# colmap/privacy_preserving_sfm

Hardware: AMD Instinct MI355X
Metric: BA iterations/sec + RANSAC hypotheses/sec, 500 cams / 200k line obs (higher is better)
Workload: dtype f64; 1 GPU; configs[2]: 500 cams / 200k line obs full BA (K1+K2+K3, MFMA Schur solve) on 1xMI355X; cams=500, points=25000, obs=200000, camera_model=SIMPLE_RADIAL, reduced_system=3000, successful_steps=2561, lm_chunk=10, submodels=1, exchange=none (independent sub-models), linear_solver=cholesky (one launch: chain workgroup + task list), cholesky_fallbacks=0

## Files before the change

### privacy_preserving_sfm_amd/csrc/chol_block.hpp

```cpp
#pragma once
#include <type_traits>
#include <utility>

#include "ba_impl.hpp"

namespace ppsfm {

constexpr int kNB = 64;
constexpr int kDeferAbove = 280;
constexpr int kNumCUs = 256;
constexpr int kPanelThreads = 1024;
typedef double v4f64 __attribute__((ext_vector_type(4)));

#ifdef PP_CHOL_TRACE
__device__ long long g_chol_trace[32];
__device__ long long g_chol_trace2[32][128];
__device__ int g_chol_step;
#define PP_CHOL_PHASE(i) do { if (threadIdx.x == 0 && blockIdx.x == 0) { const long long t_ = wall_clock64(); g_chol_trace[i] = t_; g_chol_trace2[i][g_chol_step & 127] = t_; } } while (0)
#define PP_CHOL_STAMP(i) do { if (threadIdx.x == 0) g_chol_trace[i] = wall_clock64(); } while (0)
__device__ int g_chol_exp;
#define PP_EXP(bit) (g_chol_exp & (bit))
__device__ long long g_wave_arrive[12][16];
__device__ long long g_bs_trace[5][128];
#define PP_BS_STAMP(slot, blk) do { if (threadIdx.x == 0) g_bs_trace[slot][(blk) & 127] = wall_clock64(); } while (0)
// ... 3 lines not shown
#define PP_CHOL_LAUNCH(slot, k) do { if (threadIdx.x == 0 && (k) < 64) atomicMax((unsigned long long*)&g_chol_launch[slot][k], (unsigned long long)wall_clock64()); } while (0)
__device__ int g_chol_skip;
#define PP_CHOL_SKIPPED(bit) (g_chol_skip & (1 << (bit)))
__device__ long long g_task_trace[24][128];
__device__ int g_dbg_mismatch[16];
__device__ int g_burn_stop;
__device__ unsigned g_burn_hwid[512];
__device__ long long g_spare_wait[3][128];
__device__ unsigned long long g_wait_missing[128];
__device__ long long g_chain_phase[8][128];
__device__ long long g_chain_clk[128];
#define PP_CHAIN_PHASE(slot, k) do { if (threadIdx.x == 0 && (k) < 128) { g_chain_phase[slot][k] = wall_clock64(); if ((slot) == 0) g_chain_clk[k] = clock64(); } } while (0)
#define PP_TASK_MAX(slot, k) do { if (threadIdx.x == 0 && (k) < 128) atomicMax((unsigned long long*)&g_task_trace[slot][k], (unsigned long long)wall_clock64()); } while (0)
#define PP_TASK_MIN(slot, k) do { if (threadIdx.x == 0 && (k) < 128) atomicMin((unsigned long long*)&g_task_trace[slot][k], (unsigned long long)wall_clock64()); } while (0)
#ifdef PP_CHOL_NO_STAMPS
#undef PP_CHOL_PHASE
#undef PP_CHOL_STAMP
#undef PP_WAVE_ARRIVE
#undef PP_CHOL_LAUNCH
#undef PP_CHAIN_PHASE
#undef PP_TASK_MAX
#undef PP_TASK_MIN
#define PP_TASK_MAX(slot, k) do { } while (0)
#define PP_TASK_MIN(slot, k) do { } while (0)
#define PP_CHAIN_PHASE(slot, k) do { } while (0)
#define PP_CHOL_LAUNCH(slot, k) do { } while (0)
#define PP_CHOL_PHASE(i) do { } while (0)
#define PP_CHOL_STAMP(i) do { } while (0)
#define PP_WAVE_ARRIVE(b) do { } while (0)
#endif
#else
#define PP_BS_STAMP(slot, blk) do { } while (0)
#define PP_TASK_MAX(slot, k) do { } while (0)
#define PP_TASK_MIN(slot, k) do { } while (0)
#define PP_CHAIN_PHASE(slot, k) do { } while (0)
#define PP_CHOL_LAUNCH(slot, k) do { } while (0)
#define PP_CHOL_SKIPPED(bit) false
#define PP_CHOL_PHASE(i) do { } while (0)
#define PP_CHOL_STAMP(i) do { } while (0)
#define PP_WAVE_ARRIVE(b) do { } while (0)
#define PP_EXP(bit) false
#endif

__device__ __forceinline__ double ReadLane(double v, int src_lane) {
  int lo = __double2loint(v), hi = __double2hiint(v);
  lo = __builtin_amdgcn_readlane(lo, src_lane);
  hi = __builtin_amdgcn_readlane(hi, src_lane);
  return __hiloint2double(hi, lo);
}

__device__ __forceinline__ v4f64 MfmaK16(const double (&a)[16], const double (&b)[16], v4f64 acc) {
  v4f64 p1 = (v4f64){0.0, 0.0, 0.0, 0.0}, p2 = p1, p3 = p1;
#pragma unroll
  for (int kk = 0; kk < 4; ++kk) {
    acc = __builtin_amdgcn_mfma_f64_16x16x4f64(a[kk], b[kk], acc, 0, 0, 0);
    p1 = __builtin_amdgcn_mfma_f64_16x16x4f64(a[4 + kk], b[4 + kk], p1, 0, 0, 0);
    p2 = __builtin_amdgcn_mfma_f64_16x16x4f64(a[8 + kk], b[8 + kk], p2, 0, 0, 0);
    p3 = __builtin_amdgcn_mfma_f64_16x16x4f64(a[12 + kk], b[12 + kk], p3, 0, 0, 0);
  }
  return (acc + p1) + (p2 + p3);
}
__device__ __forceinline__ v4f64 MfmaK4(const double (&a)[4], const v4f64& b, v4f64 acc) {
  const v4f64 z = (v4f64){0.0, 0.0, 0.0, 0.0};
  const v4f64 p0 = __builtin_amdgcn_mfma_f64_16x16x4f64(a[0], b[0], acc, 0, 0, 0);
  const v4f64 p1 = __builtin_amdgcn_mfma_f64_16x16x4f64(a[1], b[1], z, 0, 0, 0);
  const v4f64 p2 = __builtin_amdgcn_mfma_f64_16x16x4f64(a[2], b[2], z, 0, 0, 0);
  const v4f64 p3 = __builtin_amdgcn_mfma_f64_16x16x4f64(a[3], b[3], z, 0, 0, 0);
  return (p0 + p1) + (p2 + p3);
}

__device__ __forceinline__ double RsqrtPositive(double d) {
  const double r = __builtin_amdgcn_rsq(d);
  const double e = fma(-d * r, r, 1.0);
  return fma(r * e, fma(e, 0.375, 0.5), r);
}

constexpr int kLS = kNB + 2;

template <int P>
__device__ __forceinline__ void PotrfPanel16(double* A, double* inv_diag, int lane, int32_t* flag) {
  constexpr int c0 = 16 * P;
  double a[16];
#pragma unroll
  for (int jj = 0; jj < 16; ++jj) a[jj] = A[lane * kLS + c0 + jj];
  double invs[16];
#pragma unroll
  for (int jj = 0; jj < 16; ++jj) {
    const double d = ReadLane(a[jj], c0 + jj);
    const double inv = RsqrtPositive(d);
    a[jj] *= inv;
    invs[jj] = inv;
#pragma unroll
    for (int cc = jj + 1; cc < 16; ++cc) {
      const double s = ReadLane(a[jj], c0 + cc);
      a[cc] = fma(-a[jj], s, a[cc]);
    }
  }
  if (lane == 0) {
#pragma unroll
    for (int jj = 0; jj < 16; ++jj) inv_diag[c0 + jj] = invs[jj];
    if (!(invs[15] < 1.7976931348623157e308)) atomicOr(flag, 1);
  }
  if (lane >= c0) {
#pragma unroll
    for (int jj = 0; jj < 16; ++jj) A[lane * kLS + c0 + jj] = a[jj];
  }
}

template <int N>
__device__ __forceinline__ double RowBroadcast(double v) {
  double r;
  asm("s_nop 1\n\tv_mov_b64_dpp %0, %1 row_newbcast:%2 row_mask:0xf bank_mask:0xf" : "=v"(r) : "v"(v), "n"(N));
  return r;
}
__device__ __forceinline__ double ScaleForBroadcast(double v, double s) {
  double r;
  asm("v_mul_f64 %0, %1, %2\n\ts_nop 1" : "=v"(r) : "v"(v), "v"(s));
  return r;
}
template <int N, bool kFreshSource = false>
__device__ __forceinline__ void SubMulRowBroadcast(double& acc, double bsrc, double own) {
  if (kFreshSource) asm("s_nop 1\n\tv_fmac_f64_dpp %0, -%1, %2 row_newbcast:%3 row_mask:0xf bank_mask:0xf" : "+v"(acc) : "v"(bsrc), "v"(own), "n"(N));
  else asm("v_fmac_f64_dpp %0, -%1, %2 row_newbcast:%3 row_mask:0xf bank_mask:0xf" : "+v"(acc) : "v"(bsrc), "v"(own), "n"(N));
}
template <int JJ, int... CC>
__device__ __forceinline__ double LastPanelColumn(double (&t)[16], double (&x)[16], std::integer_sequence<int, CC...>) {
  const double inv = RsqrtPositive(RowBroadcast<JJ>(t[JJ]));
  t[JJ] = ScaleForBroadcast(t[JJ], inv);
  x[JJ] *= inv;
  ((SubMulRowBroadcast<JJ + 1 + CC>(t[JJ + 1 + CC], t[JJ], t[JJ]), SubMulRowBroadcast<JJ + 1 + CC>(x[JJ + 1 + CC], t[JJ], x[JJ])), ...);
  return inv;
}
template <int... JJ>
__device__ __forceinline__ double LastPanelColumns(double (&t)[16], double (&x)[16], std::integer_sequence<int, JJ...>) {
  double inv = 0.0;
  ((inv = LastPanelColumn<JJ>(t, x, std::make_integer_sequence<int, 15 - JJ>())), ...);
  return inv;
}
__device__ __forceinline__ void PotrfLastPanelWithInverse(double* A, double* M, int lane, int32_t* flag) {
  constexpr int c0 = 48;
  const int r = lane & 15;
  double t[16], x[16];
#pragma unroll
  for (int jj = 0; jj < 16; ++jj) { t[jj] = A[(c0 + r) * kLS + c0 + jj]; x[jj] = (r == jj) ? 1.0 : 0.0; }
  const double last_inv = LastPanelColumns(t, x, std::make_integer_sequence<int, 16>());
  if (lane < 16) {
#pragma unroll
    for (int jj = 0; jj < 16; ++jj) { A[(c0 + r) * kLS + c0 + jj] = t[jj]; M[(c0 + jj) * kLS + c0 + r] = x[jj]; }
  }
  if (lane == 0 && !(last_inv < 1.7976931348623157e308)) atomicOr(flag, 1);
}

template <int Q, int... R>
__device__ __forceinline__ void InverseStep(const double (&a)[16], double (&x)[16], double inv_q, std::integer_sequence<int, R...>) {
  x[Q] *= inv_q;
  (SubMulRowBroadcast<Q + 1 + R, R == 0>(x[Q + 1 + R], a[Q], x[Q]), ...);
}
template <int... Q>
__device__ __forceinline__ void InverseSteps(const double (&a)[16], double (&x)[16], const double (&inv)[16], std::integer_sequence<int, Q...>) {
  (InverseStep<Q>(a, x, inv[Q], std::make_integer_sequence<int, 15 - Q>()), ...);
}
template <int P>
__device__ __forceinline__ void InverseDiag16(const double* A, const double* inv_diag, double* M, int lane) {
  constexpr int t0 = 16 * P;
  const int r = lane & 15;
  double a[16], x[16], inv[16];
#pragma unroll
  for (int q = 0; q < 16; ++q) { a[q] = A[(t0 + r) * kLS + t0 + q]; inv[q] = inv_diag[t0 + q]; x[q] = (q == r) ? 1.0 : 0.0; }
  InverseSteps(a, x, inv, std::make_integer_sequence<int, 16>());
  if (lane < 16) {
#pragma unroll
    for (int q = 0; q < 16; ++q) M[(t0 + q) * kLS + t0 + r] = x[q];
  }
}

__device__ __forceinline__ v4f64 TileMulAB(const double* At, const double* Bt, v4f64 acc, int lr, int g) {
  double av[4];
  v4f64 bv;
#pragma unroll
  for (int kk = 0; kk < 4; ++kk) { av[kk] = At[lr * kLS + 4 * kk + g]; bv[kk] = Bt[(4 * kk + g) * kLS + lr]; }
  return MfmaK4(av, bv, acc);
}
__device__ __forceinline__ v4f64 TileMulABt(const double* At, const double* Bt, v4f64 acc, int lr, int g) {
  double av[4];
  v4f64 bv;
#pragma unroll
  for (int kk = 0; kk < 4; ++kk) { av[kk] = At[lr * kLS + 4 * kk + g]; bv[kk] = Bt[lr * kLS + 4 * kk + g]; }
  return MfmaK4(av, bv, acc);
}
__device__ __forceinline__ v4f64 TileNegMulAD(const double* At, const v4f64& d, int lr, int g) {
  double av[4];
#pragma unroll
  for (int kk = 0; kk < 4; ++kk) av[kk] = -At[lr * kLS + 4 * kk + g];
  return MfmaK4(av, d, (v4f64){0.0, 0.0, 0.0, 0.0});
}
__device__ __forceinline__ void TileStoreD(double* Ct, const v4f64& c, int lr, int g) {
#pragma unroll
  for (int i = 0; i < 4; ++i) Ct[(g + 4 * i) * kLS + lr] = c[i];
}
#define PP_TILE(buf, ti, tj) ((buf) + (16 * (ti)) * kLS + 16 * (tj))

template <int P>
__device__ __forceinline__ void PotrfTrailing16(double* A, int lane, int w) {
  constexpr int ntile = (3 - P) * (4 - P) / 2;
  if (w >= ntile) return;
  const int lr = lane & 15, g = lane >> 4;
  int ti = P + 1, rem = w;
  while (rem > ti - (P + 1)) { rem -= ti - P; ++ti; }
  const int tj = P + 1 + rem;
  v4f64 acc;
#pragma unroll
  for (int i = 0; i < 4; ++i) acc[i] = PP_TILE(A, ti, tj)[(g + 4 * i) * kLS + lr];
  double av[4];
  v4f64 bv;
#pragma unroll
  for (int kk = 0; kk < 4; ++kk) { av[kk] = -PP_TILE(A, ti, P)[lr * kLS + 4 * kk + g]; bv[kk] = PP_TILE(A, tj, P)[lr * kLS + 4 * kk + g]; }
  acc = MfmaK4(av, bv, acc);
  TileStoreD(PP_TILE(A, ti, tj), acc, lr, g);
}

__device__ __forceinline__ double2 TileLoad2(const double* __restrict__ src, int ld, int tid, int it) {
  const int idx = tid + kPanelThreads * it, r = idx >> 5, c2 = idx & 31;
  return *reinterpret_cast<const double2*>(src + (size_t)r * ld + 2 * c2);
}
__device__ __forceinline__ void TileStore2(double* dst, int tid, int it, double2 v) {
  const int idx = tid + kPanelThreads * it, r = idx >> 5, c2 = idx & 31;
  *reinterpret_cast<double2*>(dst + r * kLS + 2 * c2) = v;
}
__device__ __forceinline__ double LoadCoherent(const double* p) { return __hip_atomic_load(p, __ATOMIC_RELAXED, __HIP_MEMORY_SCOPE_AGENT); }
__device__ __forceinline__ double2 TileLoad2Coherent(const double* __restrict__ src, int ld, int tid, int it) {
  const int idx = tid + kPanelThreads * it, r = idx >> 5, c2 = idx & 31;
  const double* p = src + (size_t)r * ld + 2 * c2;
  return make_double2(LoadCoherent(p), LoadCoherent(p + 1));
}
__device__ __forceinline__ void LoadTile(double* dst, const double* __restrict__ src, int ld, int tid) {
  const double2 a0 = TileLoad2(src, ld, tid, 0), a1 = TileLoad2(src, ld, tid, 1);
  TileStore2(dst, tid, 0, a0); TileStore2(dst, tid, 1, a1);
}
__device__ __forceinline__ void LoadTiles2(double* d0, const double* __restrict__ s0, double* d1, const double* __restrict__ s1, int ld, int tid) {
  const double2 a0 = TileLoad2(s0, ld, tid, 0), a1 = TileLoad2(s0, ld, tid, 1), b0 = TileLoad2(s1, ld, tid, 0), b1 = TileLoad2(s1, ld, tid, 1);
  TileStore2(d0, tid, 0, a0); TileStore2(d0, tid, 1, a1); TileStore2(d1, tid, 0, b0); TileStore2(d1, tid, 1, b1);
}
__device__ __forceinline__ void LoadTiles4(double* d0, const double* __restrict__ s0, double* d1, const double* __restrict__ s1, double* d2,
                                           const double* __restrict__ s2, double* d3, const double* __restrict__ s3, int ld, int tid) {
  const double2 a0 = TileLoad2(s0, ld, tid, 0), a1 = TileLoad2(s0, ld, tid, 1), b0 = TileLoad2(s1, ld, tid, 0), b1 = TileLoad2(s1, ld, tid, 1);
  const double2 c0 = TileLoad2(s2, ld, tid, 0), c1 = TileLoad2(s2, ld, tid, 1), e0 = TileLoad2(s3, ld, tid, 0), e1 = TileLoad2(s3, ld, tid, 1);
  TileStore2(d0, tid, 0, a0); TileStore2(d0, tid, 1, a1); TileStore2(d1, tid, 0, b0); TileStore2(d1, tid, 1, b1);
  TileStore2(d2, tid, 0, c0); TileStore2(d2, tid, 1, c1); TileStore2(d3, tid, 0, e0); TileStore2(d3, tid, 1, e1);
}
__device__ __forceinline__ void StoreThrough(double* p, double v) { __hip_atomic_store(p, v, __ATOMIC_RELAXED, __HIP_MEMORY_SCOPE_AGENT); }
__device__ __forceinline__ void StoreTile(double* __restrict__ dst, const double* src, int ld, int tid) {
#pragma unroll
  for (int it = 0; it < 2; ++it) {
    const int idx = tid + kPanelThreads * it, r = idx >> 5, c2 = idx & 31;
    const double2 v = *reinterpret_cast<const double2*>(src + r * kLS + 2 * c2);
    StoreThrough(dst + (size_t)r * ld + 2 * c2, v.x);
    StoreThrough(dst + (size_t)r * ld + 2 * c2 + 1, v.y);
  }
}

constexpr unsigned long long kNotReady = 0xFFFFFFFFFFFFFFFFull;
constexpr unsigned long long kNotReadyNaN = 0x7FF8000000000000ull;

__device__ __forceinline__ void SuperTileProducts(v4f64 (&p)[2][2], const double* ar, const double* br) {
#pragma unroll
  for (int kk = 0; kk < 16; ++kk) {
    const double a0v = ar[4 * kk], a1v = ar[16 * kLS + 4 * kk], b0v = br[4 * kk], b1v = br[16 * kLS + 4 * kk];
    p[0][0] = __builtin_amdgcn_mfma_f64_16x16x4f64(a0v, b0v, p[0][0], 0, 0, 0);
    p[0][1] = __builtin_amdgcn_mfma_f64_16x16x4f64(a0v, b1v, p[0][1], 0, 0, 0);
    p[1][0] = __builtin_amdgcn_mfma_f64_16x16x4f64(a1v, b0v, p[1][0], 0, 0, 0);
    p[1][1] = __builtin_amdgcn_mfma_f64_16x16x4f64(a1v, b1v, p[1][1], 0, 0, 0);
  }
}

struct NoSideJob { __device__ void operator()(int) const {} };
template <typename Side, typename Side1, typename Spare = NoSideJob>
__device__ __forceinline__ void PotrfPanels(double* A, double* M, double* inv_diag, int32_t* __restrict__ flag, int lane, int w, Side side, Side1 side1,
                                            Spare spare = Spare()) {
  constexpr int kInvWave = kPanelThreads / 64 - 1;
  __shared__ int m22_ready;
#define PP_PANEL16(P) PotrfPanel16<P>(A, inv_diag, lane, flag)
  const int lr = lane & 15, g = lane >> 4;
  const v4f64 zero = (v4f64){0.0, 0.0, 0.0, 0.0};
  if (w == kInvWave && lane == 0) __hip_atomic_store(&m22_ready, 0, __ATOMIC_RELAXED, __HIP_MEMORY_SCOPE_WORKGROUP);
  if (w == 0) { __builtin_amdgcn_s_setprio(3); PP_PANEL16(0); }
  else side(w);
  PP_WAVE_ARRIVE(0); __syncthreads();
  PP_CHOL_PHASE(3);
  PotrfTrailing16<0>(A, lane, w);
  PP_WAVE_ARRIVE(1); __syncthreads();
  PP_CHOL_PHASE(4);
  if (w == 0) PP_PANEL16(1);
  else if (w == kInvWave) InverseDiag16<0>(A, inv_diag, M, lane);
  else side1(w);
  PP_WAVE_ARRIVE(2); __syncthreads();
  PP_CHOL_PHASE(5);
  if (!std::is_same<Spare, NoSideJob>::value && (w == 4 || (w >= 7 && w < kInvWave))) {
    PP_WAVE_ARRIVE(3); __syncthreads();
    spare(0);
    PP_WAVE_ARRIVE(4); __syncthreads();
    PP_WAVE_ARRIVE(5); __syncthreads();
    spare(1);
    PP_WAVE_ARRIVE(6); __syncthreads();
    PP_WAVE_ARRIVE(7); __syncthreads();
    spare(2);
    return;
  }
  PotrfTrailing16<1>(A, lane, w);
  PP_WAVE_ARRIVE(3); __syncthreads();
  PP_CHOL_PHASE(6);
  if (w == 0) PP_PANEL16(2);
  if (w == kInvWave) InverseDiag16<1>(A, inv_diag, M, lane);
  PP_WAVE_ARRIVE(4); __syncthreads();
  PP_CHOL_PHASE(7);
  PotrfTrailing16<2>(A, lane, w);
  if (w == 1) {
    const v4f64 t = TileMulAB(PP_TILE(A, 1, 0), PP_TILE(M, 0, 0), zero, lr, g);
    TileStoreD(PP_TILE(M, 1, 0), TileNegMulAD(PP_TILE(M, 1, 1), t, lr, g), lr, g);
  }
  PP_WAVE_ARRIVE(5); __syncthreads();
  PP_CHOL_PHASE(8);
  v4f64 t = zero;
  if (w == 0) PotrfLastPanelWithInverse(A, M, lane, flag);
  if (w == kInvWave) {
    InverseDiag16<2>(A, inv_diag, M, lane);
    if (lane == 0) __hip_atomic_store(&m22_ready, 1, __ATOMIC_RELEASE, __HIP_MEMORY_SCOPE_WORKGROUP);
  }
  if (w == 1) { t = TileMulAB(PP_TILE(A, 2, 0), PP_TILE(M, 0, 0), zero, lr, g); t = TileMulAB(PP_TILE(A, 2, 1), PP_TILE(M, 1, 0), t, lr, g); }
  if (w == 2) t = TileMulAB(PP_TILE(A, 2, 1), PP_TILE(M, 1, 1), zero, lr, g);
  if (w == 3) { t = TileMulAB(PP_TILE(A, 3, 0), PP_TILE(M, 0, 0), zero, lr, g); t = TileMulAB(PP_TILE(A, 3, 1), PP_TILE(M, 1, 0), t, lr, g); }
  if (w == 5) t = TileMulAB(PP_TILE(A, 3, 1), PP_TILE(M, 1, 1), zero, lr, g);
  if (w == 1 || w == 2 || w == 6) {
    while (__hip_atomic_load(&m22_ready, __ATOMIC_ACQUIRE, __HIP_MEMORY_SCOPE_WORKGROUP) == 0) __builtin_amdgcn_s_sleep(2);
    if (w == 6) t = TileMulAB(PP_TILE(A, 3, 2), PP_TILE(M, 2, 2), zero, lr, g);
    else TileStoreD(PP_TILE(M, 2, w - 1), TileNegMulAD(PP_TILE(M, 2, 2), t, lr, g), lr, g);
  }
  PP_WAVE_ARRIVE(6); __syncthreads();
  PP_CHOL_PHASE(9);
  if (w == 3) t = TileMulAB(PP_TILE(A, 3, 2), PP_TILE(M, 2, 0), t, lr, g);
  if (w == 5) t = TileMulAB(PP_TILE(A, 3, 2), PP_TILE(M, 2, 1), t, lr, g);
  if (w == 3 || w == 5 || w == 6) TileStoreD(PP_TILE(M, 3, w == 3 ? 0 : (w == 5 ? 1 : 2)), TileNegMulAD(PP_TILE(M, 3, 3), t, lr, g), lr, g);
  PP_WAVE_ARRIVE(7); __syncthreads();
}

__device__ __forceinline__ void ZeroTile(double* dst, int tid) {
  for (int idx = tid; idx < kNB * kLS / 2; idx += kPanelThreads) reinterpret_cast<double2*>(dst)[idx] = make_double2(0.0, 0.0);
}
__device__ __forceinline__ void ZeroTileFresh(double* dst, int tid) {
  double z = 0.0;
  asm volatile("" : "+v"(z));
  for (int idx = tid; idx < kNB * kLS / 2; idx += kPanelThreads) reinterpret_cast<double2*>(dst)[idx] = make_double2(z, z);
}

template <int NK>
__device__ __forceinline__ v4f64 SolveTileN(const double* X, const double* M, int s, int ct, int lr, int g) {
  double av[4 * NK], bv[4 * NK];
#pragma unroll
  for (int kt = 0; kt < NK; ++kt)
#pragma unroll
    for (int kk = 0; kk < 4; ++kk) { av[4 * kt + kk] = PP_TILE(X, s, kt)[lr * kLS + 4 * kk + g]; bv[4 * kt + kk] = PP_TILE(M, ct, kt)[lr * kLS + 4 * kk + g]; }
  const v4f64 z = (v4f64){0.0, 0.0, 0.0, 0.0};
  v4f64 p[4] = {z, z, z, z};
#pragma unroll
  for (int i = 0; i < 4 * NK; ++i) p[i & 3] = __builtin_amdgcn_mfma_f64_16x16x4f64(av[i], bv[i], p[i & 3], 0, 0, 0);
  return (p[0] + p[1]) + (p[2] + p[3]);
}
__device__ __forceinline__ v4f64 SolveTile(const double* X, const double* M, int s, int ct, int lr, int g) {
  switch (ct) {
    case 0: return SolveTileN<1>(X, M, s, ct, lr, g);
    case 1: return SolveTileN<2>(X, M, s, ct, lr, g);
    case 2: return SolveTileN<3>(X, M, s, ct, lr, g);
    default: return SolveTileN<4>(X, M, s, ct, lr, g);
  }
}
__device__ __forceinline__ void UpdateTileInPlace(double* X, const double* A, const double* B, int ti, int tj, int lr, int g) {
  v4f64 x;
#pragma unroll
  for (int i = 0; i < 4; ++i) x[i] = PP_TILE(X, ti, tj)[(g + 4 * i) * kLS + lr];
  double av[16], bv[16];
#pragma unroll
  for (int kk = 0; kk < 16; ++kk) { av[kk] = -A[(16 * ti + lr) * kLS + 4 * kk + g]; bv[kk] = B[(16 * tj + lr) * kLS + 4 * kk + g]; }
  x = MfmaK16(av, bv, x);
  TileStoreD(PP_TILE(X, ti, tj), x, lr, g);
}

__device__ __forceinline__ v4f64 UpdateTileRegs(v4f64 x, const double* A, const double* B, int ti, int tj, int lr, int g) {
  double av[16], bv[16];
#pragma unroll
  for (int kk = 0; kk < 16; ++kk) { av[kk] = -A[(16 * ti + lr) * kLS + 4 * kk + g]; bv[kk] = B[(16 * tj + lr) * kLS + 4 * kk + g]; }
  return MfmaK16(av, bv, x);
}


__device__ __forceinline__ void SmallFactorSolveTiles(double* tiles, double* inv_diag, double* xs, double* ys, int32_t* flag, int T, int n, double* __restrict__ x_out) {
  const int tid = threadIdx.x, lane = tid & 63, w = tid >> 6;
  double* A11 = tiles; double* A21 = tiles + kNB * kLS; double* A22 = tiles + 2 * kNB * kLS; double* Mb = tiles + 3 * kNB * kLS;
  for (int blk = 0; blk < T; ++blk) {
    double* A = blk ? A22 : A11;
    double* Md = blk ? A11 : Mb;
    if (blk) {
      const int s = w & 3, ct = w >> 2, lr = lane & 15, g = lane >> 4;
      const v4f64 x = SolveTile(A21, Mb, s, ct, lr, g);
      __syncthreads();
      TileStoreD(PP_TILE(A21, s, ct), x, lr, g);
      __syncthreads();
      if (w < 10) {
        int di = 0, rem = w;
        while (rem > di) { rem -= di + 1; ++di; }
        UpdateTileInPlace(A22, A21, A21, di, rem, lr, g);
      }
    }
    ZeroTile(Md, tid);
    __syncthreads();
    PotrfPanels(A, Md, inv_diag, flag, lane, w, NoSideJob(), NoSideJob());
  }
  const int m2 = T == 2 ? n - kNB : 0, n1 = T == 2 ? kNB : n;
  if (T == 2) {
    if (tid < m2) ys[kNB + tid] = A22[m2 * kLS + tid];
    if (tid < kNB) ys[tid] = A21[m2 * kLS + tid];
    __syncthreads();
    if (tid < m2) { double v = 0.0; for (int i = tid; i < m2; ++i) v += A11[i * kLS + tid] * ys[kNB + i]; xs[kNB + tid] = v; }
    __syncthreads();
    if (tid < kNB) { double v = ys[tid]; for (int i = 0; i < m2; ++i) v -= A21[i * kLS + tid] * xs[kNB + i]; ys[tid] = v; }
    __syncthreads();
  } else {
    if (tid < n1) ys[tid] = A11[n * kLS + tid];
    __syncthreads();
  }
  if (tid < n1) { double v = 0.0; for (int i = tid; i < n1; ++i) v += Mb[i * kLS + tid] * ys[i]; xs[tid] = v; }
  __syncthreads();
  if (tid < n) x_out[tid] = xs[tid];
  __syncthreads();
}

}
```

### privacy_preserving_sfm_amd/csrc/chol_tasks.hpp

```cpp
#pragma once
#include "chol_backsub.hpp"
#include "chol_block.hpp"
#include "chol_plan.hpp"

namespace ppsfm {

constexpr int kSpinBound = 1 << 21;

struct Mailboxes {
  double* Minv;
  double* xs;
  double* ds;
  double* xsol;
  double* Pw;
  double* Zw;
};
inline Mailboxes MailboxesOf(double* ws, const CholWorkspace& w) { return Mailboxes{ws + w.Minv, ws + w.xs, ws + w.ds, ws + w.xsol, ws + w.Pw, ws + w.Zw}; }

__device__ __forceinline__ void WaitOwnStores() { asm volatile("s_waitcnt vmcnt(0)" ::: "memory"); }
__device__ __forceinline__ void TaskStoresDone() {
  WaitOwnStores();
  __syncthreads();
}
__device__ __forceinline__ bool IsPoison(double v) { return (unsigned long long)__double_as_longlong(v) == kNotReady; }
__device__ __forceinline__ void StoreMail(double* p, double v) { StoreThrough(p, IsPoison(v) ? __longlong_as_double((long long)kNotReadyNaN) : v); }

struct WaitList {
  const int32_t *p0 = nullptr, *p1 = nullptr, *p2 = nullptr, *p3 = nullptr, *p4 = nullptr;
  int n0 = 0, n1 = 0, n2 = 0, n3 = 0, n4 = 0;
};
__device__ __forceinline__ bool TaskWait(const WaitList& wl, int32_t* flag, int* s_failed, unsigned long long* last_missing = nullptr) {
  if (threadIdx.x < 64) {
    const int l = threadIdx.x;
    const int32_t* p = l == 0 ? wl.p0 : (l == 1 ? wl.p1 : (l == 2 ? wl.p2 : (l == 3 ? wl.p3 : wl.p4)));
    const int need = l == 0 ? wl.n0 : (l == 1 ? wl.n1 : (l == 2 ? wl.n2 : (l == 3 ? wl.n3 : wl.n4)));
    bool mine = l >= 5 || need <= 0;
    for (int spins = 0;; ++spins) {
      if (last_missing && l == 0) *last_missing = __ballot(!mine) | ((unsigned long long)spins << 8);
      if (!mine) mine = __hip_atomic_load(p, __ATOMIC_RELAXED, __HIP_MEMORY_SCOPE_AGENT) >= need;
      if (__all(mine)) break;
      bool give_up = spins >= kSpinBound;
      if ((spins & 1023) == 1023) give_up = give_up || (__hip_atomic_load(flag, __ATOMIC_RELAXED, __HIP_MEMORY_SCOPE_AGENT) & 4);
      if (give_up) { if (l == 0) { atomicOr(flag, 4); *s_failed = 1; } break; }
      __builtin_amdgcn_s_sleep(1);
    }
  }
  __syncthreads();
  return *s_failed == 0;
}

struct NoDeposit { __device__ void operator()() const {} };
template <bool kEager = false, typename Deposit = NoDeposit>
__device__ __forceinline__ bool FetchMailTile(double* dst, const double* __restrict__ src, int tid, int32_t* flag, int* s_failed, Deposit deposit = Deposit()) {
  const int r0 = tid >> 5, c2 = tid & 31;
  const double* p0 = src + (size_t)r0 * kNB + 2 * c2;
  const double* p1 = p0 + (size_t)32 * kNB;
  const double* probe = src + (size_t)(tid & 63) * kNB + (((tid & 63) * 5) & 63);
  bool mine = false;
  for (int spins = 0;; ++spins) {
    if (!mine) {
      const double a = LoadCoherent(p0), b = LoadCoherent(p0 + 1), c = LoadCoherent(p1), d = LoadCoherent(p1 + 1);
      if (spins == 0) deposit();
      if (!IsPoison(a) && !IsPoison(b) && !IsPoison(c) && !IsPoison(d)) {
        *reinterpret_cast<double2*>(dst + r0 * kLS + 2 * c2) = make_double2(a, b);
        *reinterpret_cast<double2*>(dst + (r0 + 32) * kLS + 2 * c2) = make_double2(c, d);
        mine = true;
      }
    }
    if (kEager) {
      if (mine) break;
      bool give_up = spins >= kSpinBound;
      if ((spins & 1023) == 1023) give_up = give_up || (__hip_atomic_load(flag, __ATOMIC_RELAXED, __HIP_MEMORY_SCOPE_AGENT) & 4);
      if (give_up) { atomicOr(flag, 4); *s_failed = 1; break; }
      continue;
    }
    if (__syncthreads_and(mine)) break;
    if (tid < 64) {
      for (int inner = 0;; ++inner) {
        if (__all(!IsPoison(LoadCoherent(probe)))) break;
        bool give_up = inner >= kSpinBound || spins >= 4096;
        if ((inner & 1023) == 1023) give_up = give_up || (__hip_atomic_load(flag, __ATOMIC_RELAXED, __HIP_MEMORY_SCOPE_AGENT) & 4);
        if (give_up) { if (tid == 0) { atomicOr(flag, 4); *s_failed = 1; } break; }
        __builtin_amdgcn_s_sleep(1);
      }
    }
    __syncthreads();
    if (*s_failed) break;
  }
  if (kEager) __syncthreads();
  return *s_failed == 0;
}

template <typename P>
__device__ __forceinline__ P* Launder(P* p) { long long z = 0; asm volatile("" : "+s"(z)); return p + z; }

__device__ __forceinline__ void ChainLoop(double* S_, double* L_, int ld_, int T, Mailboxes mb_, int32_t* flag_, int32_t* ctr_, double* smem_, double* inv_diag_,
                                          int* s_failed, int kb, int ke, int post, int solbase) {
  int swap = 0;
  LoadTile(smem_, mb_.xs + (size_t)kb * kNB * kNB, kNB, threadIdx.x);
  LoadTile(smem_ + kNB * kLS, mb_.Minv + (size_t)kb * kNB * kNB, kNB, threadIdx.x);
  LoadTile(smem_ + 3 * kNB * kLS, S_ + (size_t)(kb + 1) * kNB * ld_ + (size_t)(kb + 1) * kNB, ld_, threadIdx.x);
  const int wave_index = __builtin_amdgcn_readfirstlane((int)threadIdx.x >> 6);
  for (int k = kb; k + 1 < ke; ++k) {
    double* S = Launder(S_); double* L = Launder(L_); int32_t* flag = Launder(flag_);
    double* smem = smem_; double* inv_diag = inv_diag_;
    double* mbM = Launder(mb_.Minv); const double* mbX = Launder(mb_.xs); const double* mbD = Launder(mb_.ds); double* mbS = Launder(mb_.xsol);
    int ld = ld_; asm volatile("" : "+s"(ld));
    int tid;
    {
      int wv = wave_index; asm volatile("" : "+s"(wv));
      int ln; asm volatile("v_mbcnt_lo_u32_b32 %0, -1, 0\n\tv_mbcnt_hi_u32_b32 %0, -1, %0" : "=v"(ln));
      tid = wv * 64 + ln;
    }
    (void)S;
    const int lane = tid & 63, w = tid >> 6, lr = lane & 15, g = lane >> 4;
    const bool dlate = w >= 5 && w < 12 && (w & 3) != 0;
    const bool dwave = w < 4 || dlate;
    int dti = w & 3, dtj = 0;
    if (dlate) { if (w < 8) { dti = w - 4; dtj = 1; } else { dti = w == 9 ? 2 : 3; dtj = w == 11 ? 3 : 2; } }
#ifdef PP_FETCH_9WAVES
    const int spare_rank = w == 4 ? 0 : w - 6;
    constexpr int kFetchWaves = 9, kFetchRounds = 4;
#else
    const int spare_rank = (w & 3) == 0 ? -1 : (w == 7 ? 0 : (w < 12 ? w - 8 : w - 9));
    constexpr int kFetchWaves = 6, kFetchRounds = 6;
#endif
    double* bufX = smem + (swap ? kNB * kLS : 0);
    double* bufM = smem + (swap ? 0 : kNB * kLS);
    double* BD = smem + 2 * kNB * kLS;
    double* BS = smem + 3 * kNB * kLS;
    PP_TASK_MAX(1, k);
#ifdef PP_CHOL_TRACE
    if (tid == 0) g_chol_step = k;
#endif
    const size_t xbase = (size_t)(k + 1) * kNB * ld + (size_t)k * kNB;
    PP_CHAIN_PHASE(0, k);
    PP_WAVE_ARRIVE(8);
    __syncthreads();
    PP_CHAIN_PHASE(1, k);
    if (*s_failed) return;
    v4f64 d = (v4f64){0.0, 0.0, 0.0, 0.0};
    if (dwave) {
#pragma unroll
      for (int i = 0; i < 4; ++i) d[i] = PP_TILE(BS, dti, dtj)[(g + 4 * i) * kLS + lr];
    }
    const int s = w & 3, ct = w >> 2;
    const v4f64 x = SolveTile(bufX, bufM, s, ct, lr, g);
    PP_WAVE_ARRIVE(9);
    __syncthreads();
    TileStoreD(PP_TILE(BS, s, ct), x, lr, g);
    if (!PP_EXP(1)) {
      double* mail = mbS + (size_t)k * kNB * kNB;
#pragma unroll
      for (int r = 0; r < 4; ++r) StoreMail(mail + (size_t)(16 * s + g + 4 * r) * kNB + 16 * ct + lr, x[r]);
    }
    PP_CHAIN_PHASE(2, k);
    PP_WAVE_ARRIVE(10);
    __syncthreads();
    PP_CHAIN_PHASE(3, k);
    ZeroTileFresh(bufX, tid);
    if (w < 4) {
      d = UpdateTileRegs(d, BS, BS, dti, dtj, lr, g);
      TileStoreD(PP_TILE(BD, dti, dtj), d, lr, g);
    }
    PP_WAVE_ARRIVE(11);
    __syncthreads();
    PP_CHAIN_PHASE(4, k);
    const bool has_next = k + 2 < ke;
    auto side = [&](int wv) {
      if (dlate) {
        if (dtj == 1) d = UpdateTileRegs(d, BS, BS, dti, dtj, lr, g);
        TileStoreD(PP_TILE(BD, dti, dtj), d, lr, g);
      } else if ((wv & 3) != 0) {
        if (!has_next && !PP_EXP(2)) {
          const int p = (wv < 4 ? wv - 1 : wv - 10) * 64 + lane;
          for (int idx = p; idx < 2048; idx += 384) {
            const int r = idx >> 5, c2 = idx & 31;
            const double2 v = *reinterpret_cast<const double2*>(BS + r * kLS + 2 * c2);
            StoreThrough(L + xbase + (size_t)r * ld + 2 * c2, v.x);
            StoreThrough(L + xbase + (size_t)r * ld + 2 * c2 + 1, v.y);
          }
        }
      }
    };
    auto side1 = [&](int) {
      if (dlate && dtj != 1) UpdateTileInPlace(BD, BS, BS, dti, dtj, lr, g);
    };
    const double* srcX = mbX + (size_t)(k + 1) * kNB * kNB;
    const double* srcD = mbD + (size_t)(k + 1) * kNB * kNB;
    int sx = 0, sd = 0;
    int stage = (has_next && spare_rank >= 0) ? 0 : 4;
    auto issue = [&](const double* src, double* dst) {
#pragma unroll
      for (int j = 0; j < kFetchRounds; ++j) {
        const int pair = spare_rank + kFetchWaves * j;
        if (pair < 32) {
          const int r = 2 * pair + (lane >> 5), c = lane & 31;
          const double* g = src + (size_t)r * kNB + 2 * c;
          const int lo = __builtin_amdgcn_readfirstlane((int)(size_t)(__attribute__((address_space(3))) void*)(dst + (2 * pair) * kLS));
          const int hi = __builtin_amdgcn_readfirstlane((int)(size_t)(__attribute__((address_space(3))) void*)(dst + (2 * pair + 1) * kLS - 64));
          unsigned long long saved;
          int saved_m0;
          asm volatile("s_mov_b64 %[sv], exec\n\t"
                       "s_mov_b32 %[m0s], m0\n\t"
                       "s_mov_b32 m0, %[lo]\n\t"
                       "s_mov_b32 exec_lo, -1\n\t"
                       "s_mov_b32 exec_hi, 0\n\t"
                       "global_load_lds_dwordx4 %[g], off sc1\n\t"
                       "s_mov_b32 m0, %[hi]\n\t"
                       "s_mov_b32 exec_lo, 0\n\t"
                       "s_mov_b32 exec_hi, -1\n\t"
                       "global_load_lds_dwordx4 %[g], off sc1\n\t"
                       "s_mov_b32 m0, %[m0s]\n\t"
                       "s_mov_b64 exec, %[sv]"
                       : [sv] "=&s"(saved), [m0s] "=&s"(saved_m0) : [g] "v"(g), [lo] "s"(lo), [hi] "s"(hi) : "memory");
        }
      }
    };
    auto arrived = [&](const double* dst) -> bool {
      asm volatile("s_waitcnt vmcnt(0)" ::: "memory");
      bool ok = true;
#pragma unroll
      for (int j = 0; j < kFetchRounds; ++j) {
        const int pair = spare_rank + kFetchWaves * j;
        if (pair < 32) {
          const int r = 2 * pair + (lane >> 5), c = lane & 31;
          const double2 v = *reinterpret_cast<const double2*>(dst + r * kLS + 2 * c);
          ok = ok && !IsPoison(v.x) && !IsPoison(v.y);
        }
      }
      return __all(ok);
    };
    auto advance = [&]() {
      if (stage == 4) return;
      const bool look_x = sx == 1, look_d = sd == 1;
      bool have_x = sx == 2, have_d = sd == 2;
      if (look_x) have_x = arrived(bufM);
      if (look_d) have_d = arrived(BS);
      if (!have_x) { issue(srcX, bufM); sx = 1; } else sx = 2;
      if (!have_d) { issue(srcD, BS); sd = 1; } else sd = 2;
      if (sx == 2 && sd == 2) stage = 4;
    };
    auto spare_job = [&](int phase) {
      if (phase < 2) { if (!PP_EXP(8)) advance(); return; }
#ifdef PP_CHOL_TRACE
      const long long wait_t0 = wall_clock64();
      const int wait_stage0 = sx * 4 + sd;
#endif
      for (int spins = 0; stage != 4; ++spins) {
        advance();
        if (stage == 4) break;
        bool give_up = spins >= kSpinBound;
        if ((spins & 255) == 255) give_up = give_up || (__hip_atomic_load(flag, __ATOMIC_RELAXED, __HIP_MEMORY_SCOPE_AGENT) & 4);
        if (give_up) { if (lane == 0) { atomicOr(flag, 4); *s_failed = 1; } break; }
      }
#ifdef PP_CHOL_TRACE
      if (w == 7 && lane == 0 && k < 128) { g_spare_wait[0][k] = wall_clock64() - wait_t0; g_spare_wait[1][k] = wait_stage0; g_spare_wait[2][k] = wait_t0; }
      if (has_next && spare_rank >= 0 && PP_EXP(16)) {
        for (int which = 0; which < 2; ++which) {
          const double* src = which ? srcD : srcX; const double* dst = which ? BS : bufM;
          for (int j = 0; j < kFetchRounds; ++j) {
            const int pair = spare_rank + kFetchWaves * j;
            if (pair < 32) {
              const int r = 2 * pair + (lane >> 5), c = lane & 31;
              const double a = dst[r * kLS + 2 * c], b = dst[r * kLS + 2 * c + 1];
              const double ga = LoadCoherent(src + (size_t)r * kNB + 2 * c), gb = LoadCoherent(src + (size_t)r * kNB + 2 * c + 1);
              if (__double_as_longlong(a) != __double_as_longlong(ga) || __double_as_longlong(b) != __double_as_longlong(gb)) atomicAdd(&g_dbg_mismatch[which * 8 + (lane >> 5) * 4 + (j & 3)], 1);
            }
          }
        }
      }
#endif
    };
    PotrfPanels(BD, bufX, inv_diag, flag, lane, w, side, side1, spare_job);
    PP_CHAIN_PHASE(5, k);
    {
      double* mail = mbM + (size_t)(k + 1) * kNB * kNB;
#pragma unroll
      for (int it = 0; it < 2 && !PP_EXP(4); ++it) {
        const int idx = tid + kPanelThreads * it, r = idx >> 5, c2 = idx & 31;
        const double2 v = *reinterpret_cast<const double2*>(bufX + r * kLS + 2 * c2);
        StoreMail(mail + (size_t)r * kNB + 2 * c2, v.x);
        StoreMail(mail + (size_t)r * kNB + 2 * c2 + 1, v.y);
      }
    }
    if (k + 2 == T) StoreTile(L + xbase + kNB, BD, ld, tid);
    PP_CHAIN_PHASE(6, k);
    PP_TASK_MAX(2, k);
    swap ^= 1;
  }
  TaskStoresDone();
  if (ke < T && threadIdx.x == 0) __hip_atomic_store(ctr_ + solbase + (ke - 1), post, __ATOMIC_RELAXED, __HIP_MEMORY_SCOPE_AGENT);
}

__device__ __forceinline__ int32_t* VerCounter(int32_t* ctr, int I, int J) { return ctr + cVer0 + I * kMaxSuper + J; }

template <bool kIsX>
__device__ __forceinline__ void PrepTask(double* S, double* L, int ld, int k, Mailboxes mb, int32_t* __restrict__ flag, int32_t* __restrict__ ctr, int* s_failed,
                                         double* Ba, double* Bb, double* Bc, double* Bm, int w0, int w1, int w2, bool far_nz, bool first, int done_km1, int done_k, int solbase) {
  const int tid = threadIdx.x, lane = tid & 63, w = tid >> 6, lr = lane & 15, g = lane >> 4;
  const int ti = w >> 2, tj = w & 3, s = w & 3, ct = w >> 2;
  const bool prev = !first;
  const size_t row_k1 = (size_t)(k + 1) * kNB * ld, row_k2 = (size_t)(k + 2) * kNB * ld;
  const size_t col_km1 = (size_t)(k - 1) * kNB, col_k = (size_t)k * kNB, col_k1 = (size_t)(k + 1) * kNB, col_k2 = (size_t)(k + 2) * kNB;
  int di = 0, dj = 0;
  if (!kIsX) { int rem = w; while (rem > di) { rem -= di + 1; ++di; } dj = rem; }
  const bool has_out = kIsX || w < 10;
  const size_t obase = kIsX ? row_k2 + col_k1 + (size_t)(16 * ti) * ld + 16 * tj : row_k2 + col_k2 + (size_t)(16 * di) * ld + 16 * dj;
  PP_TASK_MAX(kIsX ? 19 : 20, k);
  if (prev) {
    WaitList wl;
    wl.p0 = VerCounter(ctr, (k + 2) >> 1, k >> 1); wl.n0 = w0;
    wl.p1 = VerCounter(ctr, (k + 2) >> 1, kIsX ? (k + 1) >> 1 : (k + 2) >> 1); wl.n1 = w1;
    wl.p3 = ctr + solbase + (k + 2); wl.n3 = kIsX ? w2 : (far_nz ? done_km1 : 0);
    if (kIsX) { wl.p2 = ctr + solbase + (k + 1); wl.n2 = done_km1; }
    if (!TaskWait(wl, flag, s_failed)) return;
  }
  PP_TASK_MAX(kIsX ? 3 : 11, k);
  v4f64 out = (v4f64){0.0, 0.0, 0.0, 0.0};
  if (has_out) {
#pragma unroll
    for (int i = 0; i < 4; ++i) out[i] = LoadCoherent(S + obase + (size_t)(g + 4 * i) * ld + lr);
  }
  const double2 c0 = TileLoad2Coherent(S + row_k2 + col_k, ld, tid, 0), c1 = TileLoad2Coherent(S + row_k2 + col_k, ld, tid, 1);
  if (prev) {
    const double2 zz = make_double2(0.0, 0.0);
    const double2 b0 = far_nz ? TileLoad2(L + row_k2 + col_km1, ld, tid, 0) : zz, b1 = far_nz ? TileLoad2(L + row_k2 + col_km1, ld, tid, 1) : zz;
    const double2 m0 = kIsX ? TileLoad2(L + row_k1 + col_km1, ld, tid, 0) : zz, m1 = kIsX ? TileLoad2(L + row_k1 + col_km1, ld, tid, 1) : zz;
    auto deposit = [&]() {
      TileStore2(Bc, tid, 0, c0); TileStore2(Bc, tid, 1, c1); TileStore2(Bb, tid, 0, b0); TileStore2(Bb, tid, 1, b1);
      if (kIsX) { TileStore2(Bm, tid, 0, m0); TileStore2(Bm, tid, 1, m1); }
    };
    if (!FetchMailTile<false>(Ba, mb.xsol + (size_t)(k - 1) * kNB * kNB, tid, flag, s_failed, deposit)) return;
    UpdateTileInPlace(Bc, Bb, Ba, ti, tj, lr, g);
    if (kIsX) out = UpdateTileRegs(out, Bb, Bm, ti, tj, lr, g);
    else if (has_out) out = UpdateTileRegs(out, Bb, Bb, di, dj, lr, g);
    __syncthreads();
  }
  PP_TASK_MAX(kIsX ? 12 : 13, k);
  if (prev) { if (!FetchMailTile<true>(Bm, mb.Minv + (size_t)k * kNB * kNB, tid, flag, s_failed)) return; }
  else { TileStore2(Bc, tid, 0, c0); TileStore2(Bc, tid, 1, c1); LoadTile(Bm, mb.Minv + (size_t)k * kNB * kNB, kNB, tid); __syncthreads(); }
  PP_TASK_MAX(kIsX ? 4 : 14, k);
  const v4f64 x = SolveTile(Bc, Bm, s, ct, lr, g);
  __syncthreads();
  TileStoreD(PP_TILE(Bc, s, ct), x, lr, g);
  if (kIsX) {
#pragma unroll
    for (int r = 0; r < 4; ++r) StoreThrough(L + row_k2 + col_k + (size_t)(16 * s + g + 4 * r) * ld + 16 * ct + lr, x[r]);
    if (!FetchMailTile<true>(Ba, mb.xsol + (size_t)k * kNB * kNB, tid, flag, s_failed)) return;
    TaskStoresDone();
    if (tid == 0) __hip_atomic_store(ctr + solbase + (k + 2), done_k, __ATOMIC_RELAXED, __HIP_MEMORY_SCOPE_AGENT);
    out = UpdateTileRegs(out, Bc, Ba, ti, tj, lr, g);
    double* mail = mb.xs + (size_t)(k + 1) * kNB * kNB;
#pragma unroll
    for (int i = 0; i < 4; ++i) StoreMail(mail + (16 * ti + g + 4 * i) * kNB + 16 * tj + lr, out[i]);
    PP_TASK_MAX(5, k);
    StoreTile(L + row_k1 + col_k, Ba, ld, tid);
    TaskStoresDone();
    if (tid == 0) __hip_atomic_store(ctr + solbase + (k + 1), done_k, __ATOMIC_RELAXED, __HIP_MEMORY_SCOPE_AGENT);
  } else {
    __syncthreads();
    double* mail = mb.ds + (size_t)(k + 1) * kNB * kNB;
    if (has_out) {
      out = UpdateTileRegs(out, Bc, Bc, di, dj, lr, g);
#pragma unroll
      for (int i = 0; i < 4; ++i) StoreMail(mail + (16 * di + g + 4 * i) * kNB + 16 * dj + lr, out[i]);
    } else {
      int ui = 0, uj = 1, rem = w - 10;
      while (rem >= 3 - ui) { rem -= 3 - ui; ++ui; }
      uj = ui + 1 + rem;
#pragma unroll
      for (int i = 0; i < 4; ++i) StoreThrough(mail + (16 * ui + g + 4 * i) * kNB + 16 * uj + lr, 0.0);
    }
    PP_TASK_MAX(6, k);
  }
}

template <bool kTwo>
__device__ __forceinline__ void UpdateSuperTile(double* S, const double* L, int ld, int kp, int T, int I, int J, double* As, double* Bs, const uint8_t* __restrict__ nz, int fresh_mask = 0, double* zpool = nullptr, const int32_t* slot = nullptr) {
  const int tid = threadIdx.x, lane = tid & 63, w = tid >> 6;
  const int lr = lane & 15, lk = lane >> 4;
  const int wi = w >> 2, wj = w & 3;
  const int k = kp + 1, bi0 = 2 * I, bj0 = 2 * J;
  const int bi = bi0 + (wi >> 1), bj = bj0 + (wj >> 1);
  const bool front = (bi == k + 1 && bj == k + 1) || (bi == k + 2 && (bj == k + 1 || bj == k + 2));
  bool valid = bi < T && bj < T && bi >= bj && bj >= k + 1 && !front;
  if (valid && nz) valid = nz[(size_t)bi * T + kp] && nz[(size_t)bj * T + kp];
  const size_t cbase = (size_t)bi * kNB * ld + (size_t)bj * kNB + (size_t)(32 * (wi & 1) + lk) * ld + 32 * (wj & 1) + lr;
  const v4f64 z = (v4f64){0.0, 0.0, 0.0, 0.0};
  v4f64 c[2][2], p[2][2] = {{z, z}, {z, z}};
  const size_t col = (size_t)kp * kNB;
  const int ra1 = bi0 + 1 < T ? bi0 + 1 : bi0, rb1 = bj0 + 1 < T ? bj0 + 1 : bj0;
  const double* s0 = L + (size_t)bi0 * kNB * ld + col; const double* s1 = L + (size_t)ra1 * kNB * ld + col;
  const double* s2 = L + (size_t)bj0 * kNB * ld + col; const double* s3 = L + (size_t)rb1 * kNB * ld + col;
  LoadTiles4(As, s0, As + kNB * kLS, s1, Bs, s2, Bs + kNB * kLS, s3, ld, tid);
  const int tq = 2 * (wi >> 1) + (wj >> 1);
  const bool fresh = (fresh_mask >> tq) & 1;
  double* Cw = S + cbase;
  size_t ldc = (size_t)ld;
  if (zpool && valid) { Cw = zpool + (size_t)slot[tq] * kNB * kNB + (size_t)(32 * (wi & 1) + lk) * kNB + 32 * (wj & 1) + lr; ldc = kNB; }
  if (valid) {
#pragma unroll
    for (int a = 0; a < 2; ++a)
#pragma unroll
      for (int b = 0; b < 2; ++b)
#pragma unroll
        for (int i = 0; i < 4; ++i) c[a][b][i] = fresh ? 0.0 : LoadCoherent(Cw + (size_t)(16 * a + 4 * i) * ldc + 16 * b);
  }
  double2 nx[kTwo ? 8 : 1];
  if (kTwo) {
#pragma unroll
    for (int it = 0; it < 2; ++it) {
      nx[it] = TileLoad2(s0 + kNB, ld, tid, it); nx[2 + it] = TileLoad2(s1 + kNB, ld, tid, it);
      nx[4 + it] = TileLoad2(s2 + kNB, ld, tid, it); nx[6 + it] = TileLoad2(s3 + kNB, ld, tid, it);
    }
  }
  __syncthreads();
  const double* ar = As + (32 * wi + lr) * kLS + lk;
  const double* br = Bs + (32 * wj + lr) * kLS + lk;
  if (valid) SuperTileProducts(p, ar, br);
  if (kTwo) {
    if (valid) {
#pragma unroll
      for (int a = 0; a < 2; ++a)
#pragma unroll
        for (int b = 0; b < 2; ++b) { c[a][b] = c[a][b] - p[a][b]; p[a][b] = z; }
    }
    __syncthreads();
#pragma unroll
    for (int it = 0; it < 2; ++it) {
      TileStore2(As, tid, it, nx[it]); TileStore2(As + kNB * kLS, tid, it, nx[2 + it]);
      TileStore2(Bs, tid, it, nx[4 + it]); TileStore2(Bs + kNB * kLS, tid, it, nx[6 + it]);
    }
    __syncthreads();
    if (valid) SuperTileProducts(p, ar, br);
  }
  if (valid) {
#pragma unroll
    for (int a = 0; a < 2; ++a)
#pragma unroll
      for (int b = 0; b < 2; ++b)
#pragma unroll
        for (int i = 0; i < 4; ++i)
          __hip_atomic_store(Cw + (size_t)(16 * a + 4 * i) * ldc + 16 * b, c[a][b][i] - p[a][b][i], __ATOMIC_RELAXED, __HIP_MEMORY_SCOPE_AGENT);
  }
}

__device__ __forceinline__ void UpdateTilesTask(double* S, const double* L, int ld, int kp, int bi, int bj0, bool valid0, bool valid1, double* At, double* Bt, bool fresh0 = false, bool fresh1 = false, double* z0 = nullptr, double* z1 = nullptr) {
  const int tid = threadIdx.x, lane = tid & 63, w = tid >> 6, lr = lane & 15, lk = lane >> 4;
  const int ti = w >> 2, tj = w & 3;
  const size_t col = (size_t)kp * kNB;
  const size_t cbase = (size_t)bi * kNB * ld + (size_t)bj0 * kNB + (size_t)(16 * ti + lk) * ld + 16 * tj + lr;
  const v4f64 z = (v4f64){0.0, 0.0, 0.0, 0.0};
  {
    const double2 a0 = TileLoad2(L + (size_t)bi * kNB * ld + col, ld, tid, 0), a1 = TileLoad2(L + (size_t)bi * kNB * ld + col, ld, tid, 1);
    double2 b0 = make_double2(0.0, 0.0), b1 = b0, e0 = b0, e1 = b0;
    if (valid0) { b0 = TileLoad2(L + (size_t)bj0 * kNB * ld + col, ld, tid, 0); b1 = TileLoad2(L + (size_t)bj0 * kNB * ld + col, ld, tid, 1); }
    if (valid1) { e0 = TileLoad2(L + (size_t)(bj0 + 1) * kNB * ld + col, ld, tid, 0); e1 = TileLoad2(L + (size_t)(bj0 + 1) * kNB * ld + col, ld, tid, 1); }
    TileStore2(At, tid, 0, a0); TileStore2(At, tid, 1, a1);
    if (valid0) { TileStore2(Bt, tid, 0, b0); TileStore2(Bt, tid, 1, b1); }
    if (valid1) { TileStore2(Bt + kNB * kLS, tid, 0, e0); TileStore2(Bt + kNB * kLS, tid, 1, e1); }
  }
  const size_t zoff = (size_t)(16 * ti + lk) * kNB + 16 * tj + lr;
  double* C0 = z0 ? z0 + zoff : S + cbase; double* C1 = z1 ? z1 + zoff : S + cbase + kNB;
  const size_t ld0 = z0 ? (size_t)kNB : (size_t)ld, ld1 = z1 ? (size_t)kNB : (size_t)ld;
  v4f64 c0 = z, c1 = z, p0 = z, p1 = z;
  if (valid0) {
#pragma unroll
    for (int i = 0; i < 4; ++i) c0[i] = fresh0 ? 0.0 : LoadCoherent(C0 + (size_t)(4 * i) * ld0);
  }
  if (valid1) {
#pragma unroll
    for (int i = 0; i < 4; ++i) c1[i] = fresh1 ? 0.0 : LoadCoherent(C1 + (size_t)(4 * i) * ld1);
  }
  __syncthreads();
// ... 209 lines not shown
```

Measured before the change: 1221 LM iterations/s.

## Double-buffer D/S tiles in Cholesky chain and drop per-step barriers

The chain workgroup's D and S tile buffers now alternate between two shared-memory slots on each step. This lets the barrier between the diagonal-tile read and the solve-tile store be removed, and some late waves skip re-storing D tiles. An optional flag also moves the spare-wave fetch in front of the last panel barrier, so the top-of-loop barrier runs only on the first step. The aim is fewer __syncthreads on the serial chain's critical path, at the cost of subtle correctness depending on the buffer-parity logic, which is partly not shown.

```diff
diff --git a/privacy_preserving_sfm_amd/csrc/chol_block.hpp b/privacy_preserving_sfm_amd/csrc/chol_block.hpp
--- a/privacy_preserving_sfm_amd/csrc/chol_block.hpp
+++ b/privacy_preserving_sfm_amd/csrc/chol_block.hpp
@@ -329,8 +329,13 @@
     PP_WAVE_ARRIVE(5); __syncthreads();
     spare(1);
     PP_WAVE_ARRIVE(6); __syncthreads();
+#ifdef PP_CHAIN_FETCH_BEHIND_PANELS
+    spare(2);
+    PP_WAVE_ARRIVE(7); __syncthreads();
+#else
     PP_WAVE_ARRIVE(7); __syncthreads();
     spare(2);
+#endif
     return;
   }
   PotrfTrailing16<1>(A, lane, w);
diff --git a/privacy_preserving_sfm_amd/csrc/chol_tasks.hpp b/privacy_preserving_sfm_amd/csrc/chol_tasks.hpp
--- a/privacy_preserving_sfm_amd/csrc/chol_tasks.hpp
+++ b/privacy_preserving_sfm_amd/csrc/chol_tasks.hpp
@@ -115,9 +115,13 @@
     (void)S;
     const int lane = tid & 63, w = tid >> 6, lr = lane & 15, g = lane >> 4;
     const bool dlate = w >= 5 && w < 12 && (w & 3) != 0;
-    const bool dwave = w < 4 || dlate;
     int dti = w & 3, dtj = 0;
     if (dlate) { if (w < 8) { dti = w - 4; dtj = 1; } else { dti = w == 9 ? 2 : 3; dtj = w == 11 ? 3 : 2; } }
+#ifdef PP_CHAIN_ONE_D_BUFFER
+    const bool dwave = w < 4 || dlate;
+#else
+    const bool dwave = w < 4 || (dlate && dtj == 1);
+#endif
 #ifdef PP_FETCH_9WAVES
     const int spare_rank = w == 4 ? 0 : w - 6;
     constexpr int kFetchWaves = 9, kFetchRounds = 4;
@@ -127,27 +131,45 @@
 #endif
     double* bufX = smem + (swap ? kNB * kLS : 0);
     double* bufM = smem + (swap ? 0 : kNB * kLS);
+#ifdef PP_CHAIN_ONE_D_BUFFER
+    constexpr bool kAlternateD = false;
     double* BD = smem + 2 * kNB * kLS;
     double* BS = smem + 3 * kNB * kLS;
+    double* Draw = BS;
+#else
+    constexpr bool kAlternateD = true;
+    double* BD = smem + (swap ? 2 : 3) * kNB * kLS;
+    double* BS = smem + (swap ? 3 : 2) * kNB * kLS;
+    double* Draw = BD;
+#endif
+#ifdef PP_CHAIN_FETCH_BEHIND_PANELS
+    constexpr bool kFetchBehindPanels = true;
+#else
+    constexpr bool kFetchBehindPanels = false;
+#endif
     PP_TASK_MAX(1, k);
 #ifdef PP_CHOL_TRACE
     if (tid == 0) g_chol_step = k;
 #endif
     const size_t xbase = (size_t)(k + 1) * kNB * ld + (size_t)k * kNB;
     PP_CHAIN_PHASE(0, k);
-    PP_WAVE_ARRIVE(8);
-    __syncthreads();
+    if (!kFetchBehindPanels || k == kb) {
+      PP_WAVE_ARRIVE(8);
+      __syncthreads();
+    }
     PP_CHAIN_PHASE(1, k);
     if (*s_failed) return;
     v4f64 d = (v4f64){0.0, 0.0, 0.0, 0.0};
     if (dwave) {
 #pragma unroll
-      for (int i = 0; i < 4; ++i) d[i] = PP_TILE(BS, dti, dtj)[(g + 4 * i) * kLS + lr];
+      for (int i = 0; i < 4; ++i) d[i] = PP_TILE(Draw, dti, dtj)[(g + 4 * i) * kLS + lr];
     }
     const int s = w & 3, ct = w >> 2;
     const v4f64 x = SolveTile(bufX, bufM, s, ct, lr, g);
-    PP_WAVE_ARRIVE(9);
-    __syncthreads();
+    if (!kAlternateD) {
+      PP_WAVE_ARRIVE(9);
+      __syncthreads();
+    }
     TileStoreD(PP_TILE(BS, s, ct), x, lr, g);
     if (!PP_EXP(1)) {
       double* mail = mbS + (size_t)k * kNB * kNB;
@@ -170,7 +192,7 @@
     auto side = [&](int wv) {
       if (dlate) {
         if (dtj == 1) d = UpdateTileRegs(d, BS, BS, dti, dtj, lr, g);
-        TileStoreD(PP_TILE(BD, dti, dtj), d, lr, g);
+        if (dtj == 1 || !kAlternateD) TileStoreD(PP_TILE(BD, dti, dtj), d, lr, g);
       } else if ((wv & 3) != 0) {
         if (!has_next && !PP_EXP(2)) {
           const int p = (wv < 4 ? wv - 1 : wv - 10) * 64 + lane;
```

Result: no change. 1213 LM iterations/s (-0.7%).
